# ChristophReich1996/Multi-StyleGAN

Measured on AMD Instinct MI355X. Metric: training images/sec (G+D step, 256^2, seq=3x2ch), higher is better.
Workload: dtype bf16

## Files before the change

multi_stylegan_amd/csrc/conv_fprop_pp.hip:

```cpp
#include "conv_dispatch.h"
#include <stdlib.h>

typedef __bf16 bf16v8 __attribute__((ext_vector_type(8)));
typedef __attribute__((address_space(3))) char* lds_t;

struct ConvParamsPP {
    int B, IH, IW, Cx, Ck, OH, OW, N, ldy;
    int kh, kw, stride, pad, in_up, pixel_shuffle, per_sample;
    long long x_bstride, w_bstride, y_bstride;
    int Mtot, n_chunks, n_iters, m_tiles, n_tiles;
    ActEpilogue act;
};

constexpr int PM = 256, PN = 256, PROW = 128;
constexpr int PSTAGE = (PM + PN) * PROW;

__device__ __forceinline__ int pswz(int row, int slot) { return row * PROW + ((slot ^ ((row >> 1) & 7)) << 4); }
#ifdef MSG_PP_STAMPS
__device__ unsigned long long g_pp_stamps[256 * 8 * 10];
#define PP_STAMP(k) do { if (t == 8 && blockIdx.x + 256 >= gridDim.x && blockIdx.z == gridDim.z - 1 && lane == 0) { unsigned long long tt; \
    asm volatile("s_memtime %0\n\ts_waitcnt lgkmcnt(0)" : "=s"(tt) :: "memory"); \
    g_pp_stamps[((blockIdx.x + 256 - gridDim.x) * 8 + wid_u) * 10 + (k)] = tt; } } while (0)
extern "C" int msg_pp_debug_read(void* host_dst, int nbytes) {
    return hipMemcpyFromSymbol(host_dst, HIP_SYMBOL(g_pp_stamps), nbytes) == hipSuccess ? 0 : -1;
}
__device__ unsigned long long g_pp_clock[256 * 8 * 8];
#define PP_CLOCK(k) do { if (blockIdx.x + 256 >= gridDim.x && blockIdx.z == gridDim.z - 1 && lane == 0) { unsigned long long tc, tr; \
    asm volatile("s_memtime %0\n\ts_memrealtime %1\n\ts_waitcnt lgkmcnt(0)" : "=s"(tc), "=s"(tr) :: "memory"); \
    const unsigned cl_ = blockIdx.x + 256 - gridDim.x; \
    g_pp_clock[(cl_ * 8 + wid_u) * 8 + 2 * (k)] = tc; g_pp_clock[(cl_ * 8 + wid_u) * 8 + 2 * (k) + 1] = tr; } } while (0)
__device__ unsigned long long g_pp_period[256 * 8 * 16];
#define PP_PERIOD() do { if (t >= 8 && t < 24 && blockIdx.x + 256 >= gridDim.x && blockIdx.z == gridDim.z - 1 && lane == 0) { unsigned long long tt; \
    asm volatile("s_memtime %0\n\ts_waitcnt lgkmcnt(0)" : "=s"(tt) :: "memory"); \
    g_pp_period[((blockIdx.x + 256 - gridDim.x) * 8 + wid_u) * 16 + (t - 8)] = tt; } } while (0)
extern "C" int msg_pp_period_read(void* host_dst, int nbytes) {
    return hipMemcpyFromSymbol(host_dst, HIP_SYMBOL(g_pp_period), nbytes) == hipSuccess ? 0 : -1;
}
extern "C" int msg_pp_clock_read(void* host_dst, int nbytes) {
    return hipMemcpyFromSymbol(host_dst, HIP_SYMBOL(g_pp_clock), nbytes) == hipSuccess ? 0 : -1;
}
#else
#define PP_STAMP(k) do {} while (0)
#define PP_CLOCK(k) do {} while (0)
#define PP_PERIOD() do {} while (0)
#endif
#define PP_BARRIER() do { __builtin_amdgcn_sched_barrier(0); asm volatile("s_barrier" ::: "memory"); \
                          __builtin_amdgcn_sched_barrier(0); } while (0)

__global__ __launch_bounds__(512, 2) void conv_fprop_pp_kernel(const bf16_t* __restrict__ x, const bf16_t* __restrict__ w,
                                                               bf16_t* __restrict__ y, const float* __restrict__ bias,
                                                               ConvParamsPP p) {
    constexpr int VEC = 8, BKE = 64, ESZ = 2;
    __shared__ __attribute__((aligned(16))) char smem[2 * PSTAGE];

    const int tid = threadIdx.x, lane = tid & 63, wid = tid >> 6;
    const int wid_u = __builtin_amdgcn_readfirstlane(wid);
    const int grp = wid_u >> 2;
    const int wn = wid_u & 3;
    const int lr = lane & 31, lh = lane >> 5;
    const unsigned L = xcd_remap(blockIdx.x, gridDim.x);
    const int n0 = (int)(L % p.n_tiles) * PN;
    const int m0 = (int)(L / p.n_tiles) * PM;
    const int bz = blockIdx.z;
    PP_CLOCK(0);

    const int slot_phys = lane & 7;
    const int row0 = wid * 32 + (lane >> 3);
    const int sw0 = (row0 >> 1) & 7;
    const int ohw = p.OH * p.OW;
    const int taps = p.kh * p.kw;
    const msg_desc_t d_x = msg_make_desc((const char*)x + (p.per_sample ? (long long)bz * p.x_bstride * ESZ : 0));
    const msg_desc_t d_w = msg_make_desc((const char*)w + (p.per_sample ? (long long)bz * p.w_bstride * ESZ : 0));
    const unsigned lds0 = (unsigned)(unsigned long long)(lds_t)smem;
    unsigned rc[4];
#pragma unroll
    for (int j = 0; j < 4; ++j) {
        const int m = m0 + row0 + 8 * j;
        const bool ok = m < p.Mtot;
        const int mm = ok ? m : 0;
        const int b = p.per_sample ? 0 : mm / ohw;
        const int pix = p.per_sample ? mm : mm - b * ohw;
        const int oh = pix / p.OW, ow = pix - oh * p.OW;
        rc[j] = (ok ? 0u : 0x80000000u) | ((unsigned)b << 22) | ((unsigned)oh << 11) | (unsigned)ow;
    }
    int va[4], vb[4];
#pragma unroll
    for (int j = 0; j < 4; ++j) {
        const int n = n0 + row0 + 8 * j;
        const int sl = slot_phys ^ (sw0 ^ ((j & 1) << 2));
        vb[j] = n < p.N ? (int)(((long long)n * taps * p.Ck + sl * VEC) * ESZ) : MSG_DMA_OOB;
        va[j] = MSG_DMA_OOB;
    }
    const bool ragged = (p.Cx % BKE) != 0;
    int ld_tap = -1, ld_chunk = p.n_chunks - 1, ld_tile = -1;
    auto advance = [&]() __attribute__((always_inline)) {
        if (++ld_tile >= p.n_iters) {
#pragma unroll
            for (int j = 0; j < 4; ++j) { va[j] = MSG_DMA_OOB; vb[j] = MSG_DMA_OOB; }
            ld_chunk = 0;
            ld_tap = taps;
            return;
        }
        if (++ld_chunk == p.n_chunks) {
            ld_chunk = 0;
            ++ld_tap;
            const int kh_ = ld_tap / p.kw, kw_ = ld_tap - kh_ * p.kw;
#pragma unroll
            for (int j = 0; j < 4; ++j) {
                const int sl = slot_phys ^ (sw0 ^ ((j & 1) << 2));
                bool ok = (rc[j] >> 31) == 0;
                const int b = p.per_sample ? 0 : (int)((rc[j] >> 22) & 0x1ff);
                const int oh = (int)((rc[j] >> 11) & 0x7ff), ow = (int)(rc[j] & 0x7ff);
                int ih = oh * p.stride - p.pad + kh_, iw = ow * p.stride - p.pad + kw_;
                ok = ok & (ih >= 0) & (iw >= 0);
                if (p.in_up > 1) {
                    ok = ok & (ih % p.in_up == 0) & (iw % p.in_up == 0);
                    ih /= p.in_up; iw /= p.in_up;
                }
                ok = ok & (ih < p.IH) & (iw < p.IW);
                va[j] = ok ? (int)(((long long)b * p.x_bstride + ((long long)ih * p.IW + iw) * p.Cx + sl * VEC) * ESZ) : MSG_DMA_OOB;
            }
        }
    };
    auto dma_a = [&](int j, int stage) __attribute__((always_inline)) {
        const bool c_bad = ragged && (ld_chunk * BKE + (slot_phys ^ (sw0 ^ ((j & 1) << 2))) * VEC + VEC > p.Cx);
        msg_dma16(d_x, lds0 + stage * PSTAGE + (wid_u * 32 + 8 * j) * PROW, c_bad ? MSG_DMA_OOB : va[j], ld_chunk * PROW);
    };
    auto dma_b = [&](int j, int stage) __attribute__((always_inline)) {
        msg_dma16(d_w, lds0 + stage * PSTAGE + PM * PROW + (wid_u * 32 + 8 * j) * PROW, vb[j], min(ld_tile, p.n_iters) * PROW);
    };
    auto issue = [&](int jlo, int stage) __attribute__((always_inline)) {
#pragma unroll
        for (int jj = 0; jj < 2; ++jj) { dma_a(jlo + jj, stage); dma_b(jlo + jj, stage); }
    };
    auto issue_one = [&](int j, bool b_rows, int stage) __attribute__((always_inline)) {
        if (!b_rows) dma_a(j, stage); else dma_b(j, stage);
    };

    f32x16 acc[4][2];
#pragma unroll
    for (int i = 0; i < 4; ++i)
#pragma unroll
        for (int j = 0; j < 2; ++j)
#pragma unroll
            for (int e = 0; e < 16; ++e) acc[i][j][e] = 0.f;

    bf16v8 fa[2][4], fb[2][4];
    unsigned fa_addr[4], fb_addr[4];
    {
        const unsigned sw = (unsigned)(lr >> 1) & 7u;
#pragma unroll
        for (int ks = 0; ks < 4; ++ks) {
            const unsigned koff = (((unsigned)(2 * ks + lh)) ^ sw) << 4;
            fa_addr[ks] = (unsigned)((grp * 128 + lr) * PROW) + koff;
            fb_addr[ks] = (unsigned)(PM * PROW + (wn * 64 + lr) * PROW) + koff;
        }
    }
    auto read_half = [&](int h) __attribute__((always_inline)) {
#pragma unroll
        for (int ks = 0; ks < 4; ++ks)
#pragma unroll
            for (int t = 0; t < 2; ++t) {
                fa[t][ks] = *reinterpret_cast<const bf16v8*>(smem + fa_addr[ks] + (h * 64 + t * 32) * PROW);
                fb[t][ks] = *reinterpret_cast<const bf16v8*>(smem + fb_addr[ks] + (t * 32) * PROW);
            }
    };
    auto flip_stage = [&]() __attribute__((always_inline)) {
#pragma unroll
        for (int ks = 0; ks < 4; ++ks) { fa_addr[ks] ^= (unsigned)PSTAGE; fb_addr[ks] ^= (unsigned)PSTAGE; }
    };
    auto mfma_half = [&](int h, bool dma, int stage) __attribute__((always_inline)) {
#pragma unroll
        for (int ks = 0; ks < 4; ++ks) {
#pragma unroll
            for (int i = 0; i < 2; ++i)
#pragma unroll
                for (int j = 0; j < 2; ++j)
                    acc[h * 2 + i][j] = __builtin_amdgcn_mfma_f32_32x32x16_bf16(fb[j][ks], fa[i][ks], acc[h * 2 + i][j], 0, 0, 0);
            if (dma) issue_one(2 + (ks >> 1), (ks & 1) != 0, stage);
        }
    };

    const int T = p.n_iters;
    advance();
    issue(0, 0);
    issue(2, 0);
    asm volatile("s_waitcnt vmcnt(0)" ::: "memory");
    PP_BARRIER();
    if (grp == 1) PP_BARRIER();

    PP_CLOCK(1);
    for (int t = 0; t < T; ++t) {
        const int buf = t & 1;
        PP_PERIOD();
        PP_STAMP(0);
        if (t + 1 < T) { advance(); issue(0, buf ^ 1); issue(2, buf ^ 1); }
        PP_STAMP(1);
        read_half(0);
        asm volatile("s_waitcnt lgkmcnt(0)" ::: "memory");
        PP_STAMP(2);
        PP_BARRIER();
        PP_STAMP(3);
        __builtin_amdgcn_s_setprio(1);
        mfma_half(0, false, 0);
        __builtin_amdgcn_s_setprio(0);
        PP_STAMP(4);
        PP_BARRIER();
        PP_STAMP(5);
        read_half(1);
        flip_stage();
        asm volatile("s_waitcnt lgkmcnt(0)" ::: "memory");
        PP_STAMP(6);
        if (grp == 1) asm volatile("s_waitcnt vmcnt(0)" ::: "memory");
        PP_STAMP(7);
        PP_BARRIER();
        PP_STAMP(8);
        __builtin_amdgcn_s_setprio(1);
        mfma_half(1, false, 0);
        __builtin_amdgcn_s_setprio(0);
        if (grp == 0) asm volatile("s_waitcnt vmcnt(0)" ::: "memory");
        PP_STAMP(9);
        PP_BARRIER();
    }
    if (grp == 0) PP_BARRIER();
    PP_CLOCK(2);

    constexpr int PITCH = 64 * ESZ;
    char* ep = smem + wid * (128 * PITCH);
#pragma unroll
    for (int j = 0; j < 2; ++j)
#pragma unroll
        for (int g = 0; g < 4; ++g) {
            const int unit = 8 * j + 2 * g + lh;
            float bv[4] = {0.f, 0.f, 0.f, 0.f};
            if (bias) {
                const int nb = n0 + wn * 64 + 4 * unit;
#pragma unroll
                for (int e = 0; e < 4; ++e) bv[e] = nb + e < p.N ? bias[nb + e] : 0.f;
            }
#pragma unroll
            for (int i = 0; i < 4; ++i) {
                const int row = i * 32 + lr;
                uint2 pk;
                pk.x = (unsigned)f2bf(acc[i][j][4 * g + 0] + bv[0]) | ((unsigned)f2bf(acc[i][j][4 * g + 1] + bv[1]) << 16);
                pk.y = (unsigned)f2bf(acc[i][j][4 * g + 2] + bv[2]) | ((unsigned)f2bf(acc[i][j][4 * g + 3] + bv[3]) << 16);
                *reinterpret_cast<uint2*>(ep + row * PITCH + ((unit ^ (row & 15)) << 3)) = pk;
            }
        }
    const int er = lane >> 3, ec = (lane & 7) * VEC;
    const int n = n0 + wn * 64 + ec;
    int nn = n, q = 0;
    if (p.pixel_shuffle) { const int oc = p.N >> 2; q = n / oc; nn = n - q * oc; }
    const int lim = p.pixel_shuffle ? (p.N >> 2) - nn : p.N - n;
    const bool n_ok = n < p.N;
    int gp[16];
    float a_bias[VEC], a_noise[16];
    {
        const int m_first = min(m0 + grp * 128 + er, p.Mtot - 1);
        int b = p.per_sample ? bz : m_first / ohw;
        const int pix0 = p.per_sample ? m_first : m_first - b * ohw;
        int oh = pix0 / p.OW, ow = pix0 - oh * p.OW;
        const bool want_noise = p.act.enabled == 1 && p.act.noise;
        const float nw = want_noise ? p.act.noise_w[0] : 0.f;
        if (p.act.enabled == 1) {
#pragma unroll
            for (int e = 0; e < VEC; ++e) a_bias[e] = (p.act.bias && n + e < p.N) ? p.act.bias[n + e] : 0.f;
        }
#pragma unroll
        for (int pass = 0; pass < 16; ++pass) {
            const bool ok = m0 + grp * 128 + pass * 8 + er < p.Mtot;
            const int pix = oh * p.OW + ow;
            const int g = p.pixel_shuffle ? ((b * 2 * p.OH + 2 * oh + (q >> 1)) * (2 * p.OW) + 2 * ow + (q & 1))
                                          : b * ohw + pix;
            gp[pass] = ok ? g : -1;
            a_noise[pass] = (want_noise && ok) ? nw * p.act.noise[(long long)(p.act.noise_batch == 1 ? 0 : b) * ohw + pix] : 0.f;
            ow += 8;
            while (ow >= p.OW) { ow -= p.OW; ++oh; }
            if (!p.per_sample) while (oh >= p.OH) { oh -= p.OH; ++b; }
        }
    }
    __syncthreads();
    u32x4 v[16];
#pragma unroll
    for (int pass = 0; pass < 16; ++pass) {
        const int row = pass * 8 + er;
        v[pass] = *reinterpret_cast<const u32x4*>(ep + row * PITCH + (((lane & 7) ^ ((row & 15) >> 1)) << 4));
    }
    if (er & 1) {
#pragma unroll
        for (int pass = 0; pass < 16; ++pass) v[pass] = u32x4{v[pass][2], v[pass][3], v[pass][0], v[pass][1]};
    }
    if (p.act.enabled == 1) {
#pragma unroll
        for (int pass = 0; pass < 16; ++pass) v[pass] = act_epilogue_apply<bf16_t>(v[pass], a_bias, a_noise[pass], p.act.alpha, p.act.scale);
    } else if (p.act.enabled == 2) {
        const bf16_t* rbase = reinterpret_cast<const bf16_t*>(p.act.residual) + (n_ok ? n : 0);
        u32x4 r[16];
#pragma unroll
        for (int pass = 0; pass < 16; ++pass)
            r[pass] = *reinterpret_cast<const u32x4*>(rbase + (long long)max(gp[pass], 0) * p.act.res_ld);
#pragma unroll
        for (int pass = 0; pass < 16; ++pass) v[pass] = residual_epilogue_apply<bf16_t>(v[pass], r[pass], p.act.res_gain);
    }
    bf16_t* ybase = y + (p.pixel_shuffle ? nn : n);
    if (n_ok && lim >= VEC) {
#pragma unroll
        for (int pass = 0; pass < 16; ++pass)
            if (gp[pass] >= 0) *reinterpret_cast<u32x4*>(ybase + (long long)gp[pass] * p.ldy) = v[pass];
    } else if (n_ok) {
#pragma unroll
        for (int pass = 0; pass < 16; ++pass) {
            if (gp[pass] < 0) continue;
            bf16_t* dst = ybase + (long long)gp[pass] * p.ldy;
            for (int e = 0; e < lim; ++e) dst[e] = (bf16_t)(v[pass][e >> 1] >> (16 * (e & 1)));
        }
    }
    PP_CLOCK(3);
}

bool conv_pp_eligible(const ConvProblem& q, ConvPlan* plan) {
    static const int enabled = msg_tunable("MSG_CONV_PP", 1);
    if (!enabled || q.dtype != MSG_BF16) return false;
    const long long mtot = q.mtot();
    const int N = q.N, n_iters = q.kh * q.kw * (q.Ck / 64);
    if (N < 256 || mtot < 1024 || n_iters < 4 || mtot >= (1ll << 31)) return false;
    if ((long long)((N + PN - 1) / PN) * PN * 100 > (long long)N * 115) return false;
    if ((long long)(n_iters + 1) * PROW + 128 > 65536) return false;
    if (!q.fits31()) return false;
    const long long blocks = ((mtot + PM - 1) / PM) * ((N + PN - 1) / PN);
    if (blocks >= (1ll << 31)) return false;
    if (blocks * q.samples() < 224) return false;
    *plan = ConvPlan{CONV_PP, PM, PN, true};
    return true;
}

void conv_pp_launch(const ConvProblem& q, const ConvPlan&, const void* x, const void* w, const float* bias, void* y,
                    const ActEpilogue* act, void* stream) {
    ConvParamsPP p{};
    conv_fill_common(p, q, act);
    conv_fill_taps(p, q);
    p.n_chunks = q.Ck / 64;
    p.n_iters = q.kh * q.kw * p.n_chunks;
    p.m_tiles = (int)((q.mtot() + PM - 1) / PM);
    p.n_tiles = (q.N + PN - 1) / PN;
    dim3 grid((unsigned)((long long)p.m_tiles * p.n_tiles), 1, q.samples());
    hipLaunchKernelGGL(conv_fprop_pp_kernel, grid, dim3(512), 0, (hipStream_t)stream, (const bf16_t*)x, (const bf16_t*)w,
                       (bf16_t*)y, bias, p);
}
```

multi_stylegan_amd/csrc/msg_common.h:

```cpp
#pragma once
#include <hip/hip_runtime.h>
#include <hip/hip_bf16.h>
#include <stdint.h>
#include <stdlib.h>
#include "../../include/msg_hip.h"

#ifdef MSG_TUNING
static inline int msg_tunable(const char* name, int dflt) { const char* e = getenv(name); return e ? atoi(e) : dflt; }
#else
#define msg_tunable(name, dflt) (dflt)
#endif

typedef float  f32x4 __attribute__((ext_vector_type(4)));
typedef float  f32x16 __attribute__((ext_vector_type(16)));
typedef short  bf16x8 __attribute__((ext_vector_type(8)));
typedef short  bf16x4 __attribute__((ext_vector_type(4)));
typedef unsigned short bf16_t;
typedef _Float16 f16_t;
typedef unsigned int u32x4 __attribute__((ext_vector_type(4)));

__device__ __forceinline__ float bf2f(bf16_t v) { return __uint_as_float(((uint32_t)v) << 16); }
__device__ __forceinline__ bf16_t f2bf(float f) {
    __hip_bfloat16 h = __float2bfloat16(f);
    return *reinterpret_cast<bf16_t*>(&h);
}

template <typename T> struct Vec16;
template <> struct Vec16<float> {
    static constexpr int N = 4;
    uint4 raw;
    __device__ __forceinline__ void zero() { raw = make_uint4(0, 0, 0, 0); }
    __device__ __forceinline__ float get(int i) const { return __uint_as_float((&raw.x)[i]); }
    __device__ __forceinline__ void set(int i, float v) { (&raw.x)[i] = __float_as_uint(v); }
};
template <> struct Vec16<bf16_t> {
    static constexpr int N = 8;
    uint4 raw;
    __device__ __forceinline__ void zero() { raw = make_uint4(0, 0, 0, 0); }
    __device__ __forceinline__ float get(int i) const {
        uint32_t w = (&raw.x)[i >> 1];
        return (i & 1) ? __uint_as_float(w & 0xffff0000u) : __uint_as_float(w << 16);
    }
    __device__ __forceinline__ void set2(int pair, float lo, float hi) {
        (&raw.x)[pair] = (uint32_t)f2bf(lo) | ((uint32_t)f2bf(hi) << 16);
    }
};

template <> struct Vec16<f16_t> {
    static constexpr int N = 8;
    uint4 raw;
    __device__ __forceinline__ void zero() { raw = make_uint4(0, 0, 0, 0); }
    __device__ __forceinline__ float get(int i) const {
        const uint32_t w = (&raw.x)[i >> 1];
        const unsigned short h = (unsigned short)((i & 1) ? (w >> 16) : (w & 0xffffu));
        return (float)__builtin_bit_cast(_Float16, h);
    }
    __device__ __forceinline__ void set2(int pair, float lo, float hi) {
        const unsigned short a = __builtin_bit_cast(unsigned short, (_Float16)lo);
        const unsigned short b = __builtin_bit_cast(unsigned short, (_Float16)hi);
        (&raw.x)[pair] = (uint32_t)a | ((uint32_t)b << 16);
    }
};

template <typename T> __device__ __forceinline__ float load_as_f32(const T* p);
template <> __device__ __forceinline__ float load_as_f32<float>(const float* p) { return *p; }
template <> __device__ __forceinline__ float load_as_f32<bf16_t>(const bf16_t* p) { return bf2f(*p); }
template <> __device__ __forceinline__ float load_as_f32<f16_t>(const f16_t* p) { return (float)*p; }
template <typename T> __device__ __forceinline__ void store_from_f32(T* p, float v);
template <> __device__ __forceinline__ void store_from_f32<f16_t>(f16_t* p, float v) { *p = (f16_t)v; }
template <> __device__ __forceinline__ void store_from_f32<float>(float* p, float v) { *p = v; }
template <> __device__ __forceinline__ void store_from_f32<bf16_t>(bf16_t* p, float v) { *p = f2bf(v); }

__device__ __forceinline__ unsigned xcd_remap(unsigned bid, unsigned nblk) {
    const unsigned q = nblk >> 3, r = nblk & 7u, x = bid & 7u;
    const unsigned base = (x < r) ? x * (q + 1) : r * (q + 1) + (x - r) * q;
    return base + (bid >> 3);
}

__device__ __forceinline__ float wave_sum(float v) {
#pragma unroll
    for (int off = 32; off > 0; off >>= 1) v += __shfl_xor(v, off, 64);
    return v;
}

struct ActEpilogue {
    const float* bias;
    const float* noise;
    const float* noise_w;
    int noise_batch;
    int enabled;
    float alpha, scale;
    const void* residual;
    int res_ld;
    float res_gain;
    unsigned char* mask;
    int mask_tile_m, mask_tile_n;
    const void* sign_src;
    int sign_ld;
    float* part_b;
    float* part_n;
};

__device__ __host__ __forceinline__ long long act_mask_index(long long q, int cv, int C, int tile_m, int tile_n) {
    const int vpt = tile_n >> 3;
    const long long tm = q / tile_m;
    const int r = (int)(q - tm * tile_m), tn = cv / vpt, c = cv - tn * vpt;
    return ((tm * (C / tile_n) + tn) * tile_m + r) * vpt + c;
}

__device__ __forceinline__ unsigned int act_sign_byte(u32x4 packed) {
    unsigned int t = 0;
    const unsigned int ones = 0x00010001u;
#pragma unroll
    for (int k = 0; k < 4; ++k) {
        unsigned int h;
#if defined(__HIP_DEVICE_COMPILE__)
        asm("v_pk_max_i16 %0, %1, 0\n\tv_pk_min_u16 %0, %0, %2" : "=&v"(h) : "v"((unsigned int)packed[k]), "s"(ones));
#else
        h = 0;
#endif
        t |= h << (2 * k);
    }
    return (t | (t >> 15)) & 0xffu;
}

template <typename T>
__device__ __forceinline__ u32x4 residual_epilogue_apply(u32x4 raw, u32x4 res, float gain) {
    constexpr int VEC = 16 / sizeof(T);
    Vec16<T> v, r, o;
    v.raw = make_uint4(raw[0], raw[1], raw[2], raw[3]);
    r.raw = make_uint4(res[0], res[1], res[2], res[3]);
    float f[VEC];
#pragma unroll
    for (int e = 0; e < VEC; ++e) f[e] = fmaf(1.f, v.get(e), r.get(e)) * gain;
    if constexpr (VEC == 4) {
#pragma unroll
        for (int e = 0; e < 4; ++e) o.set(e, f[e]);
    } else {
#pragma unroll
        for (int e = 0; e < 4; ++e) o.set2(e, f[2 * e], f[2 * e + 1]);
    }
    u32x4 out;
    out[0] = o.raw.x; out[1] = o.raw.y; out[2] = o.raw.z; out[3] = o.raw.w;
    return out;
}

template <typename T, bool UNIT_SLOPE = false>
__device__ __forceinline__ u32x4 act_epilogue_apply(u32x4 raw, const float* bv, float nv, float alpha, float scale) {
    constexpr int VEC = 16 / sizeof(T);
    Vec16<T> v, o;
    v.raw = make_uint4(raw[0], raw[1], raw[2], raw[3]);
    float f[VEC];
#pragma unroll
    for (int e = 0; e < VEC; ++e) {
        const float add = nv + bv[e];
        const float val = v.get(e) + add;
        f[e] = (UNIT_SLOPE ? fmaxf(val, val * alpha) : ((val > 0.f) ? val : val * alpha)) * scale;
    }
    if constexpr (VEC == 4) {
#pragma unroll
        for (int e = 0; e < 4; ++e) o.set(e, f[e]);
    } else {
#pragma unroll
        for (int e = 0; e < 4; ++e) o.set2(e, f[2 * e], f[2 * e + 1]);
    }
    u32x4 r;
    r[0] = o.raw.x; r[1] = o.raw.y; r[2] = o.raw.z; r[3] = o.raw.w;
    return r;
}

typedef int msg_desc_t __attribute__((ext_vector_type(4)));
constexpr int MSG_DMA_OOB = (int)0x80000000;
__device__ __forceinline__ msg_desc_t msg_make_desc(const void* base) {
    const unsigned long long a = (unsigned long long)base;
    msg_desc_t d;
    d[0] = __builtin_amdgcn_readfirstlane((int)(unsigned)a);
    d[1] = __builtin_amdgcn_readfirstlane((int)(unsigned)((a >> 32) & 0xffffu));
    d[2] = 0x7ffffff0;
    d[3] = 0x00020000;
    return d;
}
#pragma clang diagnostic push
#pragma clang diagnostic ignored "-Winline-asm"
__device__ __forceinline__ void msg_dma16(msg_desc_t desc, unsigned lds_addr, int voff, int soff) {
#if defined(__HIP_DEVICE_COMPILE__)
    asm volatile("s_mov_b32 m0, %0\n\ts_nop 0\n\tbuffer_load_dwordx4 %1, %2, %3 offen lds"
                 :: "s"(lds_addr), "v"(voff), "s"(desc), "s"(soff) : "memory", "m0");
#endif
}
#pragma clang diagnostic pop

#define MSG_CHECK_LAUNCH() (hipGetLastError() == hipSuccess ? MSG_OK : MSG_ELAUNCH)

extern "C" int msg_bias_act_reduce_launch(const float* part_b, float* grad_bias, int C, long long n_b, const float* part_n,
                                          float* grad_nw, long long n_n, void* stream);
```

Baseline: 157.9.

## Add persistent multi-tile conv fprop kernel overlapping epilogue with next tile loads

Adds a persistent variant of the 256x256 pipelined conv fprop kernel. Each workgroup loops over several output tiles, with tiles banded per XCD, and prefetches the next tile's first stages while it runs the current tile's epilogue through a dedicated LDS patch region. It is used when the reduction loop is short (n_iters at or below a tunable threshold) and is meant to hide launch, prologue and epilogue costs for small-K convolutions. The risks are extra LDS use, which may reduce occupancy, a single workgroup per CU, and complex vmcnt accounting across tile boundaries.

```diff
diff --git a/multi_stylegan_amd/csrc/conv_fprop_pp.hip b/multi_stylegan_amd/csrc/conv_fprop_pp.hip
--- a/multi_stylegan_amd/csrc/conv_fprop_pp.hip
+++ b/multi_stylegan_amd/csrc/conv_fprop_pp.hip
@@ -9,26 +9,31 @@
     int kh, kw, stride, pad, in_up, pixel_shuffle, per_sample;
     long long x_bstride, w_bstride, y_bstride;
     int Mtot, n_chunks, n_iters, m_tiles, n_tiles;
+    int samples, persistent;
     ActEpilogue act;
 };
 
 constexpr int PM = 256, PN = 256, PROW = 128;
 constexpr int PSTAGE = (PM + PN) * PROW;
+constexpr int PPATCH = 32 * 64 * 2;
 
 __device__ __forceinline__ int pswz(int row, int slot) { return row * PROW + ((slot ^ ((row >> 1) & 7)) << 4); }
 #ifdef MSG_PP_STAMPS
+#ifndef PP_STAMP_T
+#define PP_STAMP_T 8
+#endif
 __device__ unsigned long long g_pp_stamps[256 * 8 * 10];
-#define PP_STAMP(k) do { if (t == 8 && blockIdx.x + 256 >= gridDim.x && blockIdx.z == gridDim.z - 1 && lane == 0) { unsigned long long tt; \
+#define PP_STAMP(k) do { if (t == PP_STAMP_T && blockIdx.x + 256 >= gridDim.x && blockIdx.z == gridDim.z - 1 && lane == 0) { unsigned long long tt; \
     asm volatile("s_memtime %0\n\ts_waitcnt lgkmcnt(0)" : "=s"(tt) :: "memory"); \
     g_pp_stamps[((blockIdx.x + 256 - gridDim.x) * 8 + wid_u) * 10 + (k)] = tt; } } while (0)
 extern "C" int msg_pp_debug_read(void* host_dst, int nbytes) {
     return hipMemcpyFromSymbol(host_dst, HIP_SYMBOL(g_pp_stamps), nbytes) == hipSuccess ? 0 : -1;
 }
-__device__ unsigned long long g_pp_clock[256 * 8 * 8];
+__device__ unsigned long long g_pp_clock[256 * 8 * 16];
 #define PP_CLOCK(k) do { if (blockIdx.x + 256 >= gridDim.x && blockIdx.z == gridDim.z - 1 && lane == 0) { unsigned long long tc, tr; \
     asm volatile("s_memtime %0\n\ts_memrealtime %1\n\ts_waitcnt lgkmcnt(0)" : "=s"(tc), "=s"(tr) :: "memory"); \
     const unsigned cl_ = blockIdx.x + 256 - gridDim.x; \
-    g_pp_clock[(cl_ * 8 + wid_u) * 8 + 2 * (k)] = tc; g_pp_clock[(cl_ * 8 + wid_u) * 8 + 2 * (k) + 1] = tr; } } while (0)
+    g_pp_clock[(cl_ * 8 + wid_u) * 16 + 2 * (k)] = tc; g_pp_clock[(cl_ * 8 + wid_u) * 16 + 2 * (k) + 1] = tr; } } while (0)
 __device__ unsigned long long g_pp_period[256 * 8 * 16];
 #define PP_PERIOD() do { if (t >= 8 && t < 24 && blockIdx.x + 256 >= gridDim.x && blockIdx.z == gridDim.z - 1 && lane == 0) { unsigned long long tt; \
     asm volatile("s_memtime %0\n\ts_waitcnt lgkmcnt(0)" : "=s"(tt) :: "memory"); \
@@ -62,7 +67,6 @@
     const int n0 = (int)(L % p.n_tiles) * PN;
     const int m0 = (int)(L / p.n_tiles) * PM;
     const int bz = blockIdx.z;
-    PP_CLOCK(0);
 
     const int slot_phys = lane & 7;
     const int row0 = wid * 32 + (lane >> 3);
@@ -189,41 +193,28 @@
     PP_BARRIER();
     if (grp == 1) PP_BARRIER();
 
-    PP_CLOCK(1);
     for (int t = 0; t < T; ++t) {
         const int buf = t & 1;
-        PP_PERIOD();
-        PP_STAMP(0);
         if (t + 1 < T) { advance(); issue(0, buf ^ 1); issue(2, buf ^ 1); }
-        PP_STAMP(1);
         read_half(0);
         asm volatile("s_waitcnt lgkmcnt(0)" ::: "memory");
-        PP_STAMP(2);
         PP_BARRIER();
-        PP_STAMP(3);
         __builtin_amdgcn_s_setprio(1);
         mfma_half(0, false, 0);
         __builtin_amdgcn_s_setprio(0);
-        PP_STAMP(4);
         PP_BARRIER();
-        PP_STAMP(5);
         read_half(1);
         flip_stage();
         asm volatile("s_waitcnt lgkmcnt(0)" ::: "memory");
-        PP_STAMP(6);
         if (grp == 1) asm volatile("s_waitcnt vmcnt(0)" ::: "memory");
-        PP_STAMP(7);
         PP_BARRIER();
-        PP_STAMP(8);
         __builtin_amdgcn_s_setprio(1);
         mfma_half(1, false, 0);
         __builtin_amdgcn_s_setprio(0);
         if (grp == 0) asm volatile("s_waitcnt vmcnt(0)" ::: "memory");
-        PP_STAMP(9);
         PP_BARRIER();
     }
     if (grp == 0) PP_BARRIER();
-    PP_CLOCK(2);
 
     constexpr int PITCH = 64 * ESZ;
     char* ep = smem + wid * (128 * PITCH);
@@ -315,7 +306,351 @@
             for (int e = 0; e < lim; ++e) dst[e] = (bf16_t)(v[pass][e >> 1] >> (16 * (e & 1)));
         }
     }
-    PP_CLOCK(3);
+}
+
+template <int ACT, bool BIAS>
+__global__ __launch_bounds__(512, 2) void conv_fprop_pp_tiles_kernel(const bf16_t* __restrict__ x, const bf16_t* __restrict__ w,
+                                                               bf16_t* __restrict__ y, const float* __restrict__ bias,
+                                                               ConvParamsPP p) {
+    constexpr int VEC = 8, BKE = 64, ESZ = 2;
+    __shared__ __attribute__((aligned(16))) char smem[2 * PSTAGE + 8 * PPATCH];
+
+    const int tid = threadIdx.x, lane = tid & 63, wid = tid >> 6;
+    const int wid_u = __builtin_amdgcn_readfirstlane(wid);
+    const int grp = wid_u >> 2;
+    const int wn = wid_u & 3;
+    const int lr = lane & 31, lh = lane >> 5;
+    const int tps = p.m_tiles * p.n_tiles;
+    const bool banded = p.persistent && tps >= 64 && (long long)tps * p.samples > (long long)gridDim.x;
+    int k_cur, k_stride, k_len, band0 = 0, band_n = tps;
+    if (banded) {
+        const int xcd = blockIdx.x & 7, q8 = tps >> 3, r8 = tps & 7;
+        band0 = xcd < r8 ? xcd * (q8 + 1) : r8 * (q8 + 1) + (xcd - r8) * q8;
+        band_n = q8 + (xcd < r8 ? 1 : 0);
+        k_cur = blockIdx.x >> 3; k_stride = ((int)gridDim.x - xcd + 7) >> 3; k_len = p.samples * band_n;
+    } else if (p.persistent) {
+        k_cur = blockIdx.x; k_stride = gridDim.x; k_len = p.samples * tps;
+    } else {
+        k_cur = blockIdx.z * tps + blockIdx.x; k_stride = 1; k_len = k_cur + 1;
+    }
+    if (k_cur >= k_len) return;
+    PP_CLOCK(0);
+
+    const int slot_phys = lane & 7;
+    const int row0 = wid * 32 + (lane >> 3);
+    const int sw0 = (row0 >> 1) & 7;
+    const int ohw = p.OH * p.OW;
+    const int taps = p.kh * p.kw;
+    typedef const __attribute__((address_space(4))) char* kernarg_t;
+    typedef const __attribute__((address_space(4))) ConvParamsPP* params_t;
+    auto params_again = [&]() __attribute__((always_inline)) -> params_t {
+        kernarg_t ka = (kernarg_t)__builtin_amdgcn_kernarg_segment_ptr();
+        asm volatile("" : "+s"(ka));
+        return (params_t)(ka + 4 * sizeof(void*));
+    };
+    msg_desc_t d_x, d_w;
+    const unsigned lds0 = (unsigned)(unsigned long long)(lds_t)smem;
+    unsigned rc[4];
+    int va[4], vb[4];
+    int ld_tap, ld_chunk, ld_tile;
+    int c_n0, c_m0, c_bz;
+    auto set_tile = [&](int k) __attribute__((always_inline)) {
+        const auto& p = *params_again();
+        const int z = k / band_n, i = k - z * band_n;
+        const unsigned L = banded ? (unsigned)(band0 + i) : xcd_remap((unsigned)i, (unsigned)band_n);
+        c_bz = z;
+        c_n0 = (int)(L % p.n_tiles) * PN;
+        c_m0 = (int)(L / p.n_tiles) * PM;
+        d_x = msg_make_desc((const char*)x + (p.per_sample ? (long long)z * p.x_bstride * ESZ : 0));
+        d_w = msg_make_desc((const char*)w + (p.per_sample ? (long long)z * p.w_bstride * ESZ : 0));
+        const int m_first = c_m0 + row0;
+        const int mm = m_first < p.Mtot ? m_first : 0;
+        int b = p.per_sample ? 0 : mm / ohw;
+        const int pix = p.per_sample ? mm : mm - b * ohw;
+        int oh = pix / p.OW, ow = pix - oh * p.OW;
+#pragma unroll
+        for (int j = 0; j < 4; ++j) {
+            const bool ok = m_first + 8 * j < p.Mtot;
+            rc[j] = ok ? (((unsigned)b << 22) | ((unsigned)oh << 11) | (unsigned)ow) : 0x80000000u;
+            ow += 8;
+            while (ow >= p.OW) { ow -= p.OW; ++oh; }
+            if (!p.per_sample) while (oh >= p.OH) { oh -= p.OH; ++b; }
+        }
+#pragma unroll
+        for (int j = 0; j < 4; ++j) {
+            const int n = c_n0 + row0 + 8 * j;
+            const int sl = slot_phys ^ (sw0 ^ ((j & 1) << 2));
+            vb[j] = n < p.N ? (int)(((long long)n * taps * p.Ck + sl * VEC) * ESZ) : MSG_DMA_OOB;
+            va[j] = MSG_DMA_OOB;
+        }
+        ld_tap = -1; ld_chunk = p.n_chunks - 1; ld_tile = -1;
+    };
+    const bool ragged = (p.Cx % BKE) != 0;
+    auto advance = [&]() __attribute__((always_inline)) {
+        ++ld_tile;
+        if (++ld_chunk == p.n_chunks) {
+            ld_chunk = 0;
+            ++ld_tap;
+            const int kh_ = ld_tap / p.kw, kw_ = ld_tap - kh_ * p.kw;
+#pragma unroll
+            for (int j = 0; j < 4; ++j) {
+                const int sl = slot_phys ^ (sw0 ^ ((j & 1) << 2));
+                bool ok = (rc[j] >> 31) == 0;
+                const int b = p.per_sample ? 0 : (int)((rc[j] >> 22) & 0x1ff);
+                const int oh = (int)((rc[j] >> 11) & 0x7ff), ow = (int)(rc[j] & 0x7ff);
+                int ih = oh * p.stride - p.pad + kh_, iw = ow * p.stride - p.pad + kw_;
+                ok = ok & (ih >= 0) & (iw >= 0);
+                if (p.in_up > 1) {
+                    ok = ok & (ih % p.in_up == 0) & (iw % p.in_up == 0);
+                    ih /= p.in_up; iw /= p.in_up;
+                }
+                ok = ok & (ih < p.IH) & (iw < p.IW);
+                va[j] = ok ? (int)(((long long)b * p.x_bstride + ((long long)ih * p.IW + iw) * p.Cx + sl * VEC) * ESZ) : MSG_DMA_OOB;
+            }
+        }
+    };
+    auto dma_a = [&](int j, int stage) __attribute__((always_inline)) {
+        const bool c_bad = ragged && (ld_chunk * BKE + (slot_phys ^ (sw0 ^ ((j & 1) << 2))) * VEC + VEC > p.Cx);
+        msg_dma16(d_x, lds0 + stage * PSTAGE + (wid_u * 32 + 8 * j) * PROW, c_bad ? MSG_DMA_OOB : va[j], ld_chunk * PROW);
+    };
+    auto dma_b = [&](int j, int stage) __attribute__((always_inline)) {
+        msg_dma16(d_w, lds0 + stage * PSTAGE + PM * PROW + (wid_u * 32 + 8 * j) * PROW, vb[j], ld_tile * PROW);
+    };
+    auto issue = [&](int jlo, int stage) __attribute__((always_inline)) {
+#pragma unroll
+        for (int jj = 0; jj < 2; ++jj) { dma_a(jlo + jj, stage); dma_b(jlo + jj, stage); }
+    };
+    auto issue_one = [&](int j, bool b_rows, int stage) __attribute__((always_inline)) {
+        if (!b_rows) dma_a(j, stage); else dma_b(j, stage);
+    };
+
+    f32x16 acc[4][2];
+#pragma unroll
+    for (int i = 0; i < 4; ++i)
+#pragma unroll
+        for (int j = 0; j < 2; ++j)
+#pragma unroll
+            for (int e = 0; e < 16; ++e) acc[i][j][e] = 0.f;
+
+    bf16v8 fa[2][4], fb[2][4];
+    unsigned fa_addr[4], fb_addr[4];
+    auto frag_addrs = [&](int stage) __attribute__((always_inline)) {
+        int lane_f = lane;
+        asm volatile("" : "+v"(lane_f));
+        const unsigned lr_f = lane_f & 31, lh_f = lane_f >> 5, sw = (lr_f >> 1) & 7u;
+#pragma unroll
+        for (int ks = 0; ks < 4; ++ks) {
+            const unsigned koff = (((unsigned)(2 * ks) + lh_f) ^ sw) << 4;
+            fa_addr[ks] = (unsigned)(stage * PSTAGE) + (unsigned)((grp * 128 + lr_f) * PROW) + koff;
+            fb_addr[ks] = (unsigned)(stage * PSTAGE) + (unsigned)(PM * PROW + (wn * 64 + lr_f) * PROW) + koff;
+        }
+    };
+    frag_addrs(0);
+    auto read_half = [&](int h) __attribute__((always_inline)) {
+#pragma unroll
+        for (int ks = 0; ks < 4; ++ks)
+#pragma unroll
+            for (int t = 0; t < 2; ++t) {
+                fa[t][ks] = *reinterpret_cast<const bf16v8*>(smem + fa_addr[ks] + (h * 64 + t * 32) * PROW);
+                fb[t][ks] = *reinterpret_cast<const bf16v8*>(smem + fb_addr[ks] + (t * 32) * PROW);
+            }
+    };
+    auto flip_stage = [&]() __attribute__((always_inline)) {
+#pragma unroll
+        for (int ks = 0; ks < 4; ++ks) { fa_addr[ks] ^= (unsigned)PSTAGE; fb_addr[ks] ^= (unsigned)PSTAGE; }
+    };
+    auto mfma_half = [&](int h, bool dma, int stage) __attribute__((always_inline)) {
+#pragma unroll
+        for (int ks = 0; ks < 4; ++ks) {
+#pragma unroll
+            for (int i = 0; i < 2; ++i)
+#pragma unroll
+                for (int j = 0; j < 2; ++j)
+                    acc[h * 2 + i][j] = __builtin_amdgcn_mfma_f32_32x32x16_bf16(fb[j][ks], fa[i][ks], acc[h * 2 + i][j], 0, 0, 0);
+            if (dma) issue_one(2 + (ks >> 1), (ks & 1) != 0, stage);
+        }
+    };
+
+    int e_n0, e_m0, e_bz;
+    auto epilogue = [&](bool has_next, int nstage) __attribute__((always_inline)) -> bool {
+        constexpr int PITCH = 64 * ESZ;
+        const auto& p = *params_again();
+        const int n0 = e_n0, m0 = e_m0, bz = e_bz;
+        int lane_e = lane;
+        asm volatile("" : "+v"(lane_e));
+        const int lr = lane_e & 31, lh = lane_e >> 5;
+        char* ep = smem + 2 * PSTAGE + wid_u * PPATCH;
+        const int er = lane_e >> 3, ec = (lane_e & 7) * VEC;
+        const int n = n0 + wn * 64 + ec;
+        int nn = n, q = 0;
+        if (p.pixel_shuffle) { const int oc = p.N >> 2; q = n / oc; nn = n - q * oc; }
+        const int lim = p.pixel_shuffle ? (p.N >> 2) - nn : p.N - n;
+        const bool n_ok = n < p.N;
+        int gp[16];
+        float a_bias[VEC], a_noise[16];
+        u32x4 r[16];
+        const int m_first = min(m0 + grp * 128 + er, p.Mtot - 1);
+        int b = p.per_sample ? bz : m_first / ohw;
+        const int pix0 = p.per_sample ? m_first : m_first - b * ohw;
+        int oh = pix0 / p.OW, ow = pix0 - oh * p.OW;
+        const bool want_noise = ACT == 1 && p.act.noise;
+        const float nw = want_noise ? p.act.noise_w[0] : 0.f;
+        if (ACT == 1) {
+#pragma unroll
+            for (int e = 0; e < VEC; ++e) a_bias[e] = (p.act.bias && n + e < p.N) ? p.act.bias[n + e] : 0.f;
+        }
+        bf16_t* ybase = y + (p.pixel_shuffle ? nn : n);
+        const bf16_t* rbase = reinterpret_cast<const bf16_t*>(p.act.residual) + (n_ok ? n : 0);
+        auto request = [&](int blk) __attribute__((always_inline)) {
+#pragma unroll
+            for (int pass = 4 * blk; pass < 4 * blk + 4; ++pass) {
+                const bool ok = m0 + grp * 128 + pass * 8 + er < p.Mtot;
+                const int pix = oh * p.OW + ow;
+                const int g = p.pixel_shuffle ? ((b * 2 * p.OH + 2 * oh + (q >> 1)) * (2 * p.OW) + 2 * ow + (q & 1))
+                                              : b * ohw + pix;
+                gp[pass] = ok ? g : -1;
+                a_noise[pass] = (want_noise && ok) ? nw * p.act.noise[(long long)(p.act.noise_batch == 1 ? 0 : b) * ohw + pix] : 0.f;
+                if (ACT == 2)
+                    r[pass] = *reinterpret_cast<const u32x4*>(rbase + (long long)max(gp[pass], 0) * p.act.res_ld);
+                ow += 8;
+                while (ow >= p.OW) { ow -= p.OW; ++oh; }
+                if (!p.per_sample) while (oh >= p.OH) { oh -= p.OH; ++b; }
+            }
+        };
+        request(0);
+#pragma unroll
+        for (int i = 0; i < 4; ++i) {
+#pragma unroll
+            for (int j = 0; j < 2; ++j)
+#pragma unroll
+                for (int g = 0; g < 4; ++g) {
+                    const int unit = 8 * j + 2 * g + lh;
+                    float bv[4] = {0.f, 0.f, 0.f, 0.f};
+                    if (BIAS) {
+                        const int nb = n0 + wn * 64 + 4 * unit;
+#pragma unroll
+                        for (int e = 0; e < 4; ++e) bv[e] = nb + e < p.N ? bias[nb + e] : 0.f;
+                    }
+                    uint2 pk;
+                    pk.x = (unsigned)f2bf(acc[i][j][4 * g + 0] + bv[0]) | ((unsigned)f2bf(acc[i][j][4 * g + 1] + bv[1]) << 16);
+                    pk.y = (unsigned)f2bf(acc[i][j][4 * g + 2] + bv[2]) | ((unsigned)f2bf(acc[i][j][4 * g + 3] + bv[3]) << 16);
+                    *reinterpret_cast<uint2*>(ep + lr * PITCH + ((unit ^ (lr & 15)) << 3)) = pk;
+                }
+            asm volatile("s_waitcnt lgkmcnt(0)" ::: "memory");
+            u32x4 v[4];
+#pragma unroll
+            for (int ps = 0; ps < 4; ++ps) {
+                const int row = ps * 8 + er;
+                v[ps] = *reinterpret_cast<const u32x4*>(ep + row * PITCH + (((lane_e & 7) ^ ((row & 15) >> 1)) << 4));
+            }
+            if (er & 1) {
+#pragma unroll
+                for (int ps = 0; ps < 4; ++ps) v[ps] = u32x4{v[ps][2], v[ps][3], v[ps][0], v[ps][1]};
+            }
+            if (ACT == 1) {
+#pragma unroll
+                for (int ps = 0; ps < 4; ++ps)
+                    v[ps] = act_epilogue_apply<bf16_t>(v[ps], a_bias, a_noise[4 * i + ps], p.act.alpha, p.act.scale);
+            } else if (ACT == 2) {
+#pragma unroll
+                for (int ps = 0; ps < 4; ++ps) v[ps] = residual_epilogue_apply<bf16_t>(v[ps], r[4 * i + ps], p.act.res_gain);
+            }
+            asm volatile("s_waitcnt lgkmcnt(0)" ::: "memory");
+            if (i < 3) request(i + 1);
+            if (i == 0 && has_next) { advance(); issue(0, nstage); issue(2, nstage); }
+            if (n_ok && lim >= VEC) {
+#pragma unroll
+                for (int ps = 0; ps < 4; ++ps)
+                    if (gp[4 * i + ps] >= 0) *reinterpret_cast<u32x4*>(ybase + (long long)gp[4 * i + ps] * p.ldy) = v[ps];
+            } else if (n_ok) {
+#pragma unroll
+                for (int ps = 0; ps < 4; ++ps) {
+                    if (gp[4 * i + ps] < 0) continue;
+                    bf16_t* dst = ybase + (long long)gp[4 * i + ps] * p.ldy;
+                    for (int e = 0; e < lim; ++e) dst[e] = (bf16_t)(v[ps][e >> 1] >> (16 * (e & 1)));
+                }
+            }
+        }
+        return has_next && m0 + grp * 128 + 128 <= p.Mtot && n0 + wn * 64 + 64 <= p.N && (!p.pixel_shuffle || ((p.N >> 2) & 7) == 0);
+    };
+
+    const int T = p.n_iters;
+    set_tile(k_cur);
+    e_n0 = c_n0; e_m0 = c_m0; e_bz = c_bz;
+    advance();
+    issue(0, 0);
+    issue(2, 0);
+    advance();
+    issue(0, 1);
+    issue(2, 1);
+    asm volatile("s_waitcnt vmcnt(8)" ::: "memory");
+    PP_BARRIER();
+    if (grp == 1) PP_BARRIER();
+
+    int stage = 0;
+    bool counted = false;
+    PP_CLOCK(1);
+    for (int tile_no = 0;; ++tile_no) {
+        const int k_next = k_cur + k_stride;
+        const bool has_next = k_next < k_len;
+        PP_CLOCK(4);
+        if (tile_no == 1) PP_CLOCK(3);
+        for (int t = 0; t < T; ++t) {
+            PP_PERIOD();
+            PP_STAMP(0);
+            if (t > 0 && (t + 1 < T || has_next)) { advance(); issue(0, stage ^ 1); issue(2, stage ^ 1); }
+            PP_STAMP(1);
+            read_half(0);
+            asm volatile("s_waitcnt lgkmcnt(0)" ::: "memory");
+            PP_STAMP(2);
+            PP_BARRIER();
+            PP_STAMP(3);
+            __builtin_amdgcn_s_setprio(1);
+            mfma_half(0, false, 0);
+            __builtin_amdgcn_s_setprio(0);
+            PP_STAMP(4);
+            PP_BARRIER();
+            PP_STAMP(5);
+            read_half(1);
+            flip_stage();
+            if (t == T - 2 && has_next) set_tile(k_next);
+            asm volatile("s_waitcnt lgkmcnt(0)" ::: "memory");
+            PP_STAMP(6);
+            if (grp == 1) {
+                if (t == 0 && counted) asm volatile("s_waitcnt vmcnt(16)" ::: "memory");
+                else asm volatile("s_waitcnt vmcnt(0)" ::: "memory");
+            }
+            PP_STAMP(7);
+            PP_BARRIER();
+            PP_STAMP(8);
+            __builtin_amdgcn_s_setprio(1);
+            mfma_half(1, false, 0);
+            __builtin_amdgcn_s_setprio(0);
+            if (grp == 0) {
+                if (t == 0 && counted) asm volatile("s_waitcnt vmcnt(16)" ::: "memory");
+                else asm volatile("s_waitcnt vmcnt(0)" ::: "memory");
+            }
+            PP_STAMP(9);
+            PP_BARRIER();
+            stage ^= 1;
+        }
+        PP_CLOCK(5);
+        if (tile_no == 0) PP_CLOCK(2);
+        if (grp == 0) PP_BARRIER();
+        counted = epilogue(has_next, stage ^ 1);
+        if (!has_next) break;
+#pragma unroll
+        for (int i = 0; i < 4; ++i)
+#pragma unroll
+            for (int j = 0; j < 2; ++j)
+#pragma unroll
+                for (int e = 0; e < 16; ++e) acc[i][j][e] = 0.f;
+        e_n0 = c_n0; e_m0 = c_m0; e_bz = c_bz;
+        k_cur = k_next;
+        frag_addrs(stage);
+        if (grp == 1) PP_BARRIER();
+    }
+    PP_CLOCK(6);
 }
 
 bool conv_pp_eligible(const ConvProblem& q, ConvPlan* plan) {
@@ -343,7 +678,22 @@
     p.n_iters = q.kh * q.kw * p.n_chunks;
     p.m_tiles = (int)((q.mtot() + PM - 1) / PM);
     p.n_tiles = (q.N + PN - 1) / PN;
-    dim3 grid((unsigned)((long long)p.m_tiles * p.n_tiles), 1, q.samples());
-    hipLaunchKernelGGL(conv_fprop_pp_kernel, grid, dim3(512), 0, (hipStream_t)stream, (const bf16_t*)x, (const bf16_t*)w,
-                       (bf16_t*)y, bias, p);
+    p.samples = q.samples();
+    static const int persistent = msg_tunable("MSG_PP_PERSISTENT", 24);
+    p.persistent = p.n_iters <= persistent;
+#ifndef MSG_PP_STAMPS
+    if (!p.persistent) {
+        dim3 grid1((unsigned)((long long)p.m_tiles * p.n_tiles), 1, q.samples());
+        hipLaunchKernelGGL(conv_fprop_pp_kernel, grid1, dim3(512), 0, (hipStream_t)stream, (const bf16_t*)x, (const bf16_t*)w,
+                           (bf16_t*)y, bias, p);
+        return;
+    }
+#endif
+    const long long tps = (long long)p.m_tiles * p.n_tiles, tiles = tps * p.samples;
+    const long long cus = msg_cu_count();
+    dim3 grid = p.persistent ? dim3((unsigned)(tiles < cus ? tiles : cus)) : dim3((unsigned)tps, 1, q.samples());
+    const int mode = conv_act_mode(act);
+    auto kernel = bias ? (mode == 1 ? conv_fprop_pp_tiles_kernel<1, true> : mode == 2 ? conv_fprop_pp_tiles_kernel<2, true> : conv_fprop_pp_tiles_kernel<0, true>)
+                       : (mode == 1 ? conv_fprop_pp_tiles_kernel<1, false> : mode == 2 ? conv_fprop_pp_tiles_kernel<2, false> : conv_fprop_pp_tiles_kernel<0, false>);
+    hipLaunchKernelGGL(kernel, grid, dim3(512), 0, (hipStream_t)stream, (const bf16_t*)x, (const bf16_t*)w, (bf16_t*)y, bias, p);
 }
diff --git a/multi_stylegan_amd/csrc/msg_common.h b/multi_stylegan_amd/csrc/msg_common.h
--- a/multi_stylegan_amd/csrc/msg_common.h
+++ b/multi_stylegan_amd/csrc/msg_common.h
@@ -190,6 +190,18 @@
 }
 #pragma clang diagnostic pop
 
+static inline int msg_cu_count() {
+    static int cached[64];
+    int dev = 0;
+    if (hipGetDevice(&dev) != hipSuccess || dev < 0 || dev >= 64) dev = 0;
+    int n = __atomic_load_n(&cached[dev], __ATOMIC_RELAXED);
+    if (n <= 0) {
+        if (hipDeviceGetAttribute(&n, hipDeviceAttributeMultiprocessorCount, dev) != hipSuccess || n <= 0) n = 1;
+        __atomic_store_n(&cached[dev], n, __ATOMIC_RELAXED);
+    }
+    return n;
+}
+
 #define MSG_CHECK_LAUNCH() (hipGetLastError() == hipSuccess ? MSG_OK : MSG_ELAUNCH)
 
 extern "C" int msg_bias_act_reduce_launch(const float* part_b, float* grad_bias, int C, long long n_b, const float* part_n,
```

New measurement: 158.0, median of 2. About the same (+0.1%).
